# aws/karpenter-core

Measured on AMD Instinct MI355X. Metric: pod-placement decisions/sec (Solve()), higher is better.
Workload: dtype int64

## Files before the change

include/ksolve.h:

```cpp
#ifndef KSOLVE_H
#define KSOLVE_H
#include <stddef.h>
#include <stdint.h>

#ifdef __cplusplus
extern "C" {
#endif

#define KS_MAX_KEYS 32
#define KS_MAX_RES 16
#define KS_MAX_VALUES 64
#define KS_MAX_ITSTATES 65535
#define KS_NO_BOUND_GT INT32_MIN
#define KS_NO_BOUND_LT INT32_MAX
#define KS_KEY_HOSTNAME (-2)
#define KS_KEY_NONE (-1)

#define KS_OK 0
#define KS_ERR_INVALID (-1)
#define KS_ERR_UNSUPPORTED (-2)
#define KS_ERR_DEVICE (-3)
#define KS_ERR_CAPACITY (-4)
#define KS_ERR_INTERNAL (-5)

// ... 404 lines not shown
#define KS_CAND_WHY_DO_NOT_EVICT 12
#define KS_CAND_WHY_LEFT 13
typedef struct ks_candidates_inputs {
  uint32_t n_pods, n_nodes, n_pdbs, n_keys;
  const int32_t* pod_node;
  const uint32_t* pod_ns;
  const uint32_t* pod_flags;
  const double* pod_deletion_cost;
  const int32_t* pod_priority;
  const uint8_t* pod_val;
  const uint32_t* pdb_ns;
  const int32_t* pdb_allowed;
  const uint32_t* pdb_req_off;
  const uint32_t* pdb_req_key; const uint64_t* pdb_req_mask;
  const uint32_t* node_why;
  const double* node_age_seconds;
  const int64_t* node_ttl_seconds;
  const uint32_t* node_pods_off;
  const uint32_t* node_pods;
} ks_candidates_inputs;
typedef struct ks_candidates_outputs {
  uint32_t n_candidates, n_empty;
  uint32_t* order; uint32_t* empty; uint32_t* why; int32_t* detail; uint32_t* n_node_pods; double* cost;
} ks_candidates_outputs;
int ks_consolidation_candidates_host(const ks_candidates_inputs* in, ks_candidates_outputs* out, int device, double* ms );

#define KS_METHOD_EXPIRATION 1u
#define KS_METHOD_DRIFT 2u
#define KS_METHOD_EMPTINESS 3u
#define KS_DEPROV_WHY_NOT_EXPIRED 14
#define KS_DEPROV_WHY_NOT_DRIFTED 15
#define KS_DEPROV_WHY_NOT_EMPTY 16
#define KS_DEPROV_NODE_DELETION_TIMESTAMP 1u
#define KS_DEPROV_NODE_HAS_EMPTINESS 2u
#define KS_DEPROV_NODE_EMPTINESS_UNPARSABLE 4u
#define KS_DEPROV_NODE_DRIFTED 8u
#define KS_DEPROV_NODE_ALL 15u
#define KS_DEPROV_MAX_TTL_SECONDS 9223372036ll
typedef struct ks_deprov_inputs {
  ks_candidates_inputs c;
  uint32_t method, drift_enabled;
  int64_t now_unix_nanos;
  const uint32_t* node_dflags;
  const int64_t* node_creation_unix_nanos;
  const int64_t* node_emptiness_unix_nanos;
  const int64_t* node_ttl_seconds_after_empty;
} ks_deprov_inputs;
typedef struct ks_deprov_outputs { ks_candidates_outputs c; uint32_t n_in_result, pad; } ks_deprov_outputs;
int ks_deprovisioning_candidates_host(const ks_deprov_inputs* in, ks_deprov_outputs* out, int device, double* ms );

#define KS_CAND_VALUE_OTHER 0xFFFFFFFFu
#define KS_CAND_OP_IN 0u
#define KS_CAND_OP_NOT_IN 1u
#define KS_CAND_OP_EXISTS 2u
#define KS_CAND_OP_DOES_NOT_EXIST 3u
typedef struct ks_selector_lists {
  uint32_t n_keys, n_namespaces;
  const uint32_t* key_n_values;
  const uint32_t* pod_label_off;
  const uint32_t* pod_label_key;
  const uint32_t* pod_label_val;
  const uint32_t* req_key;
  const uint32_t* req_op;
  const uint32_t* req_val_off;
  const uint32_t* req_val;
} ks_selector_lists;
int ks_consolidation_candidates_lists_host(const ks_candidates_inputs* in, const ks_selector_lists* sel, ks_candidates_outputs* out, int device, double* ms );
int ks_deprovisioning_candidates_lists_host(const ks_deprov_inputs* in, const ks_selector_lists* sel, ks_deprov_outputs* out, int device, double* ms );

int ks_launch_pick_dev(ks_dev_problem* const* ds, uint32_t n, const uint32_t* node, int32_t* out_type, int32_t* out_pair, double* out_price);

int ks_types_subset_dev(ks_dev_problem* const* ds, uint32_t n, const uint32_t* node, const uint64_t* lhs, uint32_t stride_words, uint32_t* out);

typedef struct ks_req1 { uint64_t mask; int32_t gt, lt; uint8_t present, complement; } ks_req1;
int ks_probe_intersection(const ks_req1* a, const ks_req1* b, const int32_t* value_int, uint32_t nvalues, int on_device, ks_req1* out);
int ks_probe_compatible(const ks_req1* a, const ks_req1* b, int well_known, const int32_t* value_int, uint32_t nvalues, int on_device, int* ok);

typedef struct ks_req_facts { uint64_t has_mask; int64_t len; int32_t op; uint8_t nidne, len0; } ks_req_facts;
int ks_probe_has(const ks_req1* a, const int32_t* value_int, uint32_t nvalues, int on_device, ks_req_facts* out);

const char* ks_last_error(void);
const char* ks_version(void);
uint32_t ks_rr_run_max(void);

#ifdef __cplusplus
}
#endif
#endif
```

karpenter_core_amd/csrc/ks_pack_rr.inc:

```
#define KS_RR_DECLINED 0xDEC11EDull
#ifndef KS_SIM
#undef LSYNC
#define LSYNC() asm volatile("" ::: "memory")
#endif
#ifdef KS_PROBES
#define RRP(i) do { const u64 t_ = __builtin_readcyclecounter(); rrp[(i)] += t_ - rrp_t; rrp_t = t_; } while (0)
#else
#define RRP(i) do { } while (0)
#endif
#ifndef RR_NWK
#define RR_NWK 7
#endif
#define RR_NW (RR_NWK + 1)
#define RR_NPL 8
#define RR_NWN RR_NWK
#define RR_NODES (RR_NWN * 64 * RR_NPL)
#define RR_NODE_AT(slot, wk, ln) (((slot) * RR_NWN * 64u) + (u32)(ln) * RR_NWN + (wk))
#define RR_NODE_SLOT(n) ((n) / (64u * RR_NWN))
#define RR_NODE_WV(n) (((n) % (64u * RR_NWN)) % RR_NWN + 1u)
#define RR_NODE_LANE(n) (((n) % (64u * RR_NWN)) / RR_NWN)
#define RR_NRC 64
#define RR_GW 8
#define RR_KMAX 16
#define RR_HC_ZERO (RR_GW * 256u)
// ... 283 lines not shown
      for (u32 j = tl.topo_begin; j < tl.topo_end; ++j) {
        const PlanTopo& tg = c.topo[j]; const TopoDyn& d = sh.dyn[j]; u64 options = 0;
        if (d.reg == 0 && d.pos == ~0ull) continue;
        constrained = true;
        if (tg.type == 0) {
          i32 best = INT32_MAX; int bestv = -1;
          for (u64 bits = d.reg & ND; bits; bits &= bits - 1) {
            const int dd = __builtin_ctzll(bits);
            const i32 cnt = tb.gcnt[(size_t)tg.g * 64 + dd] + tg.self;
            if ((i64)cnt - (i64)d.minc <= (i64)tg.maxskew && cnt < best) { best = cnt; bestv = dd; }
          }
          if (bestv >= 0) options = 1ull << bestv;
        } else if (tg.type == 1) {
          options = d.reg & tg.PD & d.pos;
          if (!options && tg.self) {
            KReq pd = kreq_exists();
            if (tg.pod_has) { pd.present = true; pd.complement = tl.complement; pd.mask = tl.mask; pd.gt = KS_NOGT; pd.lt = KS_NOLT; }
            const u64 I = kreq_has_mask(kreq_intersect(pd, nd, vi, nv), vi, nv);
            const u64 x = d.reg & I, y = d.reg & tg.PD;
            if (x) options |= x & (~x + 1);
            if (y) options |= y & (~y + 1);
          }
        } else options = d.reg & tg.PD & ~d.pos;
        if (!options) return -KS_WHY_TOPOLOGY;
        dom &= options;
      }
      if (constrained) {
        const KReq in = kreq_in(dom);
        if (!before.present) { if (!((tb.wellknown >> k) & 1u)) return -KS_WHY_TOPOLOGY_REQS; a = in; }
        else { const KReq mg = kreq_intersect(in, before, vi, nv); if (kreq_len0(mg) && !kreq_nidne(before)) return -KS_WHY_TOPOLOGY_REQS; a = mg; }
      }
    }
    if (a.present) tpres |= 1u << i;
    if (a.complement) tcomp |= 1u << i;
    if (kreq_differs(a, orig)) tchg |= 1u << i;
    sh.la_mask[i][lane] = a.mask;
  }
  return 2;
}

#define RR_CTX \
  RRLds& L = g_rr_lds; \
  const DevProb& P = L.P; const DevState& S = L.S; WaveShared& sh = L.sh; RRNrc& nt = L.nt; LeaderShared& ls = L.ls; FastTabs& ft = L.ft; \
  Tabs tb; \
  tb.K = UF(P.K); tb.R = UF(P.R); tb.T = UF(P.T); tb.TW = UF(P.TW); tb.GH = UF(P.GH); tb.E = UF(P.E); tb.S = UF(P.S); tb.SC = UF(P.SC); tb.n_ct = UF(P.n_ct); tb.wellknown = UF(P.wellknown_mask); tb.key_zone = (i32)UF(P.key_zone); tb.key_ct = (i32)UF(P.key_ct); \
  tb.q = (GA u64*)UF64((u64)S.q); tb.pod_node = (GA i32*)UF64((u64)S.pod_node); tb.pod_seq = (GA i32*)UF64((u64)S.pod_seq); \
  tb.rec = (GA u8*)UF64((u64)S.rec); tb.rec_stride = UF(S.rec_stride); tb.hcnt = (GA i32*)UF64((u64)S.hcnt); tb.n_alive = (GA u64*)UF64((u64)S.n_alive); tb.ge_rows = (const GA u64*)UF64((u64)P.ge_rows); \
  const u32 nP = UF(P.P), nM = UF(P.M), nC = UF(P.C), nG = UF(P.G), nMAX = UF(P.NMAX), nE = tb.E, nK = tb.K, nR = tb.R, nTW = tb.TW; \
  i64* const ge = (i64*)ks_dyn_lds; const u32 gs = UF(P.ge_max); \
  tb.key_nvalues = ft.key_nvalues; tb.value_int = ft.value_int; tb.its_fail = ft.its_fail; tb.its_inter = ft.its_inter; \
  tb.gcnt = ft.gcnt; tb.g_reg = ft.g_reg; tb.g_pos = ft.g_pos; tb.g_active = ft.g_active; tb.g_hpos = ft.g_hpos; tb.g_hzero = ft.g_hzero; tb.ge_cnt = ft.ge_cnt; tb.ge_vals = ge; tb.ge_stride = gs; \
  const GA ClsPlan* const plans = (const GA ClsPlan*)UF64((u64)P.plans); \
  const GA u32* const rrb = (const GA u32*)UF64((u64)P.rr_briefs); \
  GA u32* const rrm = (GA u32*)UF64((u64)P.rr_memo); \
  GA u64* const rr_types = (GA u64*)UF64((u64)P.rr_types); \
  const GA u32* const rr_mi = (const GA u32*)UF64((u64)P.rr_mi); \
  (void)sh; (void)nt; (void)ls; (void)nP; (void)nM; (void)nC; (void)nG; (void)nMAX; (void)nK; (void)nR; (void)nTW; (void)plans; (void)rrb; (void)rrm; (void)rr_types; (void)rr_mi; (void)ge; (void)gs

__shared__ RRLds g_rr_lds;

__device__ __forceinline__ u32 rr_run_group(const u64* items, const int lane, const u32 done, const u32 rem, u32& item0, u32& item1) {
  const bool in = (u32)lane < rem;
  const u64 ab = in ? items[done + lane] : 0ull;
  const u32 a = (u32)ab, b = (u32)(ab >> 32);
  item0 = RL(a, 0); item1 = RL(b, 0);
  const u64 diff = ~ballot64(in && a == item0 && b == item1);
  return diff ? (u32)__builtin_ctzll(diff) : 64u;
}
#define RR_ITEM_LIM(p) ((i32)(((p) >> 16) & 0x1FFu) - (i32)((((p) >> 16) & 0x100u) << 1))

__device__ __forceinline__ u32 rr_step_merge(const u64 (*stepk)[8], u64* const scratch, const int lane, const u32 rem, const u32 nE, const u64 vfy, u32& o_key, u32& o_pay, u32& kind, u32& stop_node, u32& stop_nrc, u32& o_rank) {
  const u64 v = (u32)lane < RR_NWK * 8u ? stepk[lane >> 3][lane & 7] : ~0ull;
  const u32 key = (u32)(v >> 32);
  const bool valid = key != 0xFFFFFFFFu;
  o_key = 0xFFFFFFFFu; o_pay = 0; kind = 0; stop_node = 0xFFFFFFFFu; stop_nrc = 0;
  u32 rank = 0;
  { const u32* const kw = (const u32*)&stepk[0][0];
#pragma unroll 4
    for (u32 m = 0; m < RR_NWK * 8u; ++m) rank += kw[2u * m + 1u] < key ? 1u : 0u; }
  o_rank = valid ? rank : 64u;
  const u32 nvalid = (u32)__builtin_popcountll(ballot64(valid));
  if (rem == 0) return 0;
  if (nvalid == 0) { kind = 2; return 0; }
  if (valid) scratch[rank] = (v & ~(1ull << 31)) | (((u32)lane & 7u) == 7u ? (1ull << 31) : 0ull);
  LSYNC();
  const bool in = (u32)lane < nvalid;
  const u64 sv = in ? scratch[lane] : ~0ull;
  LSYNC();
  const u32 skey = (u32)(sv >> 32), spay = (u32)sv & 0x7FFFFFFFu, node = spay & 0xFFFFu, nrc = (spay >> 16) & 0xFFu;
  const u32 b0 = RL(skey, 0) >> 22;
  const bool h_b = (skey >> 22) != b0, h_c = node >= nE && (skey >> 22) >= RR_CNTMAX, h_v = ((vfy >> nrc) & 1ull) != 0;
  const u64 hb = ballot64(in && (h_b || h_c || h_v)), sb = ballot64(in && (node < nE || (((u32)sv >> 31) & 1u)));
  const u64 cb = ballot64(in && !h_b && h_c), vb = ballot64(in && !h_b && !h_c && h_v);
  const u32 cap = min(min((u32)RR_STEP, rem), nvalid);
  u32 n = cap;
  bool by_hard = false;
  if (hb) { const u32 t = (u32)__builtin_ctzll(hb); if (t < n) { n = t; by_hard = true; } }
  if (sb) { const u32 t = (u32)__builtin_ctzll(sb) + 1u; if (t <= n) { if (t < n || by_hard) by_hard = false; n = min(n, t); } }
  if (by_hard) { kind = ((cb >> n) & 1ull) ? 4u : (((vb >> n) & 1ull) ? 3u : 0u); if (kind) { stop_node = RL(node, (int)n); stop_nrc = RL(nrc, (int)n); } }
  if ((u32)lane < n) { o_key = skey; o_pay = spay; }
  return n;
}

__device__ __attribute__((noinline)) u32 rr_step_merge_leader(const u32 sp, const int lane, const u32 rem, const u32 nE, const u64 vfy) {
  RRLds& L = g_rr_lds;
  u32 wkey, wpay, kind, snode, snrc, mrank;
  const u32 n = rr_step_merge(L.stepk[sp], L.mrg[0], lane, rem, nE, vfy, wkey, wpay, kind, snode, snrc, mrank);
  L.mrg_out[lane] = wpay;
  if (lane == 0) { L.mrg_k[0] = kind; L.mrg_k[1] = snode; L.mrg_k[2] = snrc; }
  LSYNC();
  return n;
}

__device__ __forceinline__ u32 rr_pick_decide(const u32 nE, const u32 mw, const u64 w, u32& node, u32& nrc, u32& child, u32& key) {
  node = 0xFFFFFFFFu; nrc = 0; child = 0; key = 0;
  if (w == ~0ull) return 2u;
  node = (u32)w & 0xFFFFu; nrc = ((u32)w >> 16) & 0xFFu; key = (u32)(w >> 32);
  const u64 chg = (u64)RL(mw, 2) | ((u64)RL(mw, 3) << 32), vfy = (u64)RL(mw, 4) | ((u64)RL(mw, 5) << 32);
  child = ((chg >> nrc) & 1ull) ? ((RL(mw, 8 + (int)(nrc >> 2)) >> (8u * (nrc & 3u))) & 0xFFu) : nrc;
  if (node >= nE && (key >> 22) >= RR_CNTMAX) return 4u;
  if ((vfy >> nrc) & 1ull) return 3u;
  return 0u;
}

__device__ __forceinline__ void rr_px_static(const int lane, const u32 pos, const u32 nn, const u64 gam, const GA u32* const rrm) {
  RRLds& L = g_rr_lds; const RRNrc& nt = L.nt;
  RREntry& E = L.ring[pos & (RR_RING - 1u)]; RRPx& X = L.px[pos & (RR_PX - 1u)];
  if (lane == 0) RR_LDS_STORE(&X.u[0], 0xFFFFFFFFu);
  LSYNC();
  const u32x4 we = *(const u32x4*)&E.w[48];
  const u32x4 wq = *(const u32x4*)&E.w[52];
  const u32x4 wh = *(const u32x4*)&E.w[56];
  u32x4 m0 = *(const u32x4*)&E.t1[0], m1 = *(const u32x4*)&E.t1[4];
  const bool cover = we.x == pos && wq.x == 0 && (wq.z & 1u);
  if (UF((cover && m1.z < nn) ? 1u : 0u)) {
    const u32 mi = UF(wq.y); const u32 mw = (u32)lane < 24 ? rrm[(size_t)mi * 24 + lane] : 0u;
    LSYNC(); if ((u32)lane < 32) { E.m[lane] = mw; E.t1[lane] = mw; } LSYNC();
    m0 = *(const u32x4*)&E.t1[0]; m1 = *(const u32x4*)&E.t1[4];
  }
  const bool go = UF((cover && m1.z == nn) ? 1u : 0u) != 0;
  u32 flags = RR_PX_STOP7, dg = 0, ngrp = 0, ho = 0, plainb = 0xFFFFFFFFu, dself = 0, dskew = 0, dpd = 0;
  if (go) {
    const u32 it0 = wq.w, it1 = wh.x, hr0 = wh.y, hr1 = wh.z, nr0 = wh.w;
    const bool dyn = UF(wq.z & 2u) != 0;
    const bool cnt0 = ((hr0 >> 25) & 1u) && (((hr0 >> 24) & 1u) || ((gam >> ((hr0 >> 16) & 63u)) & 1ull)), cnt1 = ((hr1 >> 25) & 1u) && (((hr1 >> 24) & 1u) || ((gam >> ((hr1 >> 16) & 63u)) & 1ull));
    const u32 ho0 = cnt0 ? (hr0 & 0xFFFFu) : RR_HC_SINK, ho1 = cnt1 ? (hr1 & 0xFFFFu) : RR_HC_SINK;
    ho = ho0 | (ho1 << 16);
    plainb = (!dyn && (it0 & 0xFFFFu) == RR_HC_ZERO && (it1 & 0xFFFFu) == RR_HC_ZERO) ? E.w[27] : 0xFFFFFFFFu;
    flags = RR_PX_GO | (dyn ? RR_PX_DYN : 0u) | ((dyn || (m0.z | m0.w) != 0) ? RR_PX_CHG : 0u) | ((ho1 == ho0 && cnt0 && cnt1) ? RR_PX_TWICE : 0u) | ((cnt0 || cnt1) ? RR_PX_HREC : 0u);
    ngrp = nr0 & 63u;
    {
      const u32 n = (u32)lane;
      const u64 acc1 = (u64)m0.x | ((u64)m0.y << 32), chg1 = (u64)m0.z | ((u64)m0.w << 32), vfy1 = (u64)m1.x | ((u64)m1.y << 32);
      const u32 cbyte = ((const u8*)&E.t1[8])[n];
      const bool a_ok = n < nn && ((acc1 >> n) & 1ull), a_vfy = (vfy1 >> n) & 1ull; const u32 a_child = ((chg1 >> n) & 1ull) ? cbyte : n;
      const u32 nkey = (nr0 >> 8) & 0xFFu;
      auto rec_of = [&](const u32 ac) -> u32 {
        const u32 npres = nt.present[ac], ncomp = nt.complement[ac]; const u64 nqm = nt.mask[nkey & (RR_KMAX - 1u)][ac];
        const bool rec = ((nr0 >> 16) & 1u) && ((gam >> ngrp) & 1ull) && ((npres >> nkey) & 1u) && !((ncomp >> nkey) & 1u) && __builtin_popcountll(nqm) == 1;
        return rec ? (1u | ((u32)__builtin_ctzll(nqm | (1ull << 63)) << 1)) : 0u; };
      const u32 r0 = rec_of(a_child & 63u);
      u32 tw = (a_child & 0xFFu) | (a_ok ? 1u << 8 : 0u) | (a_vfy ? 1u << 9 : 0u) | ((r0 & 1u) << 11) | (((r0 >> 1) & 63u) << 12);
      if (dyn) {
        const u32 dw = E.w[11], dk = (dw >> 16) & 0xFFu, dk0 = UF(L.wx[8]), dk1 = UF(L.wx[9]);
        dg = (dw >> 8) & 63u; dself = dw >> 24; dskew = E.w[19]; dpd = E.w[26];
        const u32 dks = dk == dk0 ? 0u : 1u, n1 = a_child & 63u;
        const u64 nd = L.dy_nd[dks][n1], vp = L.vpair[n];
// ... 346 lines not shown
        const u32 kind = rr_pick_decide(nE, mw, w, node, nrc, nrc_new, key);
        if (kind != 0) { stop_kind = kind; stop_node = node; break; }
        pseq = seq0 + j; phm = UF(E.w[51]); pbp = E.w;
        RRP(13);
      }
      const u32 oslot = RR_NODE_SLOT(node), owv = RR_NODE_WV(node), olane = RR_NODE_LANE(node);
      if (owv == wv) {
        const bool mine = (u32)lane == olane;
        const u32 cbw = pbp[lane];
        if (it >= 0 && mine) { const u32 pd = pbp[50]; tb.pod_node[pd] = (i32)node; tb.pod_seq[pd] = (i32)pseq; G_pod_reason[pd] = 0;
        }
        const i64 cq0 = (i64)((u64)RL(cbw, 0) | ((u64)RL(cbw, 1) << 32)), cq1 = (i64)((u64)RL(cbw, 2) | ((u64)RL(cbw, 3) << 32)), cq2 = (i64)((u64)RL(cbw, 4) | ((u64)RL(cbw, 5) << 32)), cq3 = (i64)((u64)RL(cbw, 6) | ((u64)RL(cbw, 7) << 32));
        const u32 prm = RL(cbw, 8), nhrec = RL(cbw, 17);
        const u32* const crp = C.create;
        u32 rej = 0;
#define RR_HREC_WORD(i, w) case w: { const u32 c = (n_hc[i][w] >> sh8) & 0xFFu; const u32 c2 = c == 0xFFu ? 1u : (c >= 254u ? 254u : c + 1u); if (mine) { n_hc[i][w] = (n_hc[i][w] & ~(0xFFu << sh8)) | (c2 << sh8); if (c == 0u) hzm |= 1u << (hs & 31u); } } break;
#define RR_COMMIT_SLOT(i) if (oslot == (i)) { \
          if (create) { \
            if (mine) { n_key[i] = UF(crp[0]); n_meta[i] = nrc_new | (UF(crp[1]) << 8); \
              n_room[i][0] = (i64)((u64)UF(crp[2]) | ((u64)UF(crp[3]) << 32)); n_room[i][1] = (i64)((u64)UF(crp[4]) | ((u64)UF(crp[5]) << 32)); \
              n_room[i][2] = (i64)((u64)UF(crp[6]) | ((u64)UF(crp[7]) << 32)); n_room[i][3] = (i64)((u64)UF(crp[8]) | ((u64)UF(crp[9]) << 32)); \
              n_hc[i][0] = UF(crp[10]); n_hc[i][1] = UF(crp[11]); n_hc[i][2] = UF(crp[12]); n_hc[i][3] = UF(crp[13]); n_hc[i][4] = UF(crp[14]); n_hc[i][5] = UF(crp[15]); n_hc[i][6] = UF(crp[16]); n_hc[i][7] = UF(crp[17]); } \
          } else { \
            const u32 nrc_old = RL(n_meta[i], (int)olane) & 0xFFu; \
            i64 d0 = cq0, d1 = cq1, d2 = cq2, d3 = cq3; \
            if (node >= nE && nrc_new != nrc_old) { d0 -= nt.cap[0][nrc_new] - nt.cap[0][nrc_old]; d1 -= nt.cap[1][nrc_new] - nt.cap[1][nrc_old]; d2 -= nt.cap[2][nrc_new] - nt.cap[2][nrc_old]; d3 -= nt.cap[3][nrc_new] - nt.cap[3][nrc_old]; } \
            if (mine) { \
              n_room[i][0] -= d0; n_room[i][1] -= d1; n_room[i][2] -= d2; n_room[i][3] -= d3; \
              if (node >= nE) n_key[i] = (((n_key[i] >> 22) + 1u) << 22) | ((RR_SEQMAX - pseq) << 3) | (n_key[i] & 7u); \
              n_meta[i] = nrc_new | ((((n_meta[i] >> 8) | prm) & 0xFFu) << 8); } \
          } \
          for (u32 t = 0; t < nhrec; ++t) if ((phm >> t) & 1u) {        \
            const u32 hs = RL(cbw, 28 + (int)t) & 0xFFu, sh8 = 8u * (hs & 3u); \
            switch (hs >> 2) { RR_HREC_WORD(i, 0) RR_HREC_WORD(i, 1) RR_HREC_WORD(i, 2) RR_HREC_WORD(i, 3) RR_HREC_WORD(i, 4) RR_HREC_WORD(i, 5) RR_HREC_WORD(i, 6) RR_HREC_WORD(i, 7) default: break; } \
          } \
          if (it >= 0) { RR_EVAL_SLOT(i) \
            if (nhost > 0) RR_HOST_ITEM(RR_HOST_AT_##i, hit0, hlim0) if (nhost > 1) RR_HOST_ITEM(RR_HOST_AT_##i, hit1, hlim1) if (nhost > 2) RR_HOST_ITEM(RR_HOST_AT_##i, hit2, hlim2) \
            okm = (okm & ~(1u << (i))) | (~rej & (1u << (i))); fresh = true; } }
#define RR_HOST_AT_0(w, sh, lim) RR_HOST_SLOT(0, w, sh, lim)
#define RR_HOST_AT_1(w, sh, lim) RR_HOST_SLOT(1, w, sh, lim)
#define RR_HOST_AT_2(w, sh, lim) RR_HOST_SLOT(2, w, sh, lim)
#define RR_HOST_AT_3(w, sh, lim) RR_HOST_SLOT(3, w, sh, lim)
#define RR_HOST_AT_4(w, sh, lim) RR_HOST_SLOT(4, w, sh, lim)
#define RR_HOST_AT_5(w, sh, lim) RR_HOST_SLOT(5, w, sh, lim)
#define RR_HOST_AT_6(w, sh, lim) RR_HOST_SLOT(6, w, sh, lim)
#define RR_HOST_AT_7(w, sh, lim) RR_HOST_SLOT(7, w, sh, lim)
        RR_COMMIT_SLOT(0) RR_COMMIT_SLOT(1) RR_COMMIT_SLOT(2) RR_COMMIT_SLOT(3) RR_COMMIT_SLOT(4) RR_COMMIT_SLOT(5) RR_COMMIT_SLOT(6) RR_COMMIT_SLOT(7)
        RR_HZ_FLUSH()
      }
    }
    if (run) {
      const RREntry& E = L.ring[pos0 & (RR_RING - 1u)];
      const u32 mw = E.m[lane & 31];
      do_eval(E, mw, 0u, true);
      u32 okb = okm, cur_item = 0, cur_item1 = 0;
      const u32 rbw = E.w[lane];
      const u32 rprm = RL(rbw, 8);
      const u64 rchg = (u64)RL(mw, 2) | ((u64)RL(mw, 3) << 32), rvfy = (u64)RL(mw, 4) | ((u64)RL(mw, 5) << 32);
      u32 done = 0, stepno = 0;
#ifdef KS_PROBES
      const u64 trun0 = __builtin_readcyclecounter(); u64 tx = trun0;
#define RRT(i) do { const u64 t_ = __builtin_readcyclecounter(); rrp[(i)] += t_ - tx; tx = t_; } while (0)
#else
#define RRT(i) do { } while (0)
#endif
      RRT(0);
      while (done < run) {
        u32 g_i0, g_i1;
        const u32 glen = rr_run_group(L.runitem[par], lane, done, run - done, g_i0, g_i1);
        RRT(5);
        if (g_i0 != cur_item || g_i1 != cur_item1) {
          cur_item = g_i0; cur_item1 = g_i1; nhost = (g_i0 >> 31) + (g_i1 >> 31);
          hit0 = g_i0 & 0xFFFFu; hlim0 = RR_ITEM_LIM(g_i0); hit1 = g_i1 & 0xFFFFu; hlim1 = RR_ITEM_LIM(g_i1);
          u32 rej = 0;
          if (nhost > 0) RR_HOST_ITEM(RR_HOST_ALL, hit0, hlim0)
          if (nhost > 1) RR_HOST_ITEM(RR_HOST_ALL, hit1, hlim1)
          okm = okb & ~rej;
        }
        RRT(6);
        const u32 rem = min(run - done, glen), sp = stepno & 1u;
        u32 kk[RR_NPL];
#pragma unroll
        for (int i = 0; i < RR_NPL; ++i) kk[i] = n_key[i] | (u32)(((i32)((okm >> i) & 1u)) - 1);
        u32 myk = 0xFFFFFFFFu, mypay = 0, b0 = 0;
        RRT(7);
        for (u32 r = 0; r < 8u && r < rem; ++r) {
          u32 lb = kk[0];
#pragma unroll
          for (int i = 1; i < RR_NPL; ++i) lb = min(lb, kk[i]);
          const u32 km = wave_min_u32(lb);
          if (km == 0xFFFFFFFFu) break;
          if (r == 0) b0 = km >> 22; else if ((km >> 22) != b0) break;
          const int wl = __builtin_ctzll(ballot64(lb == km));
          const u32 ws = km & 7u;
          u32 bm = 0;
#pragma unroll
          for (int i = 0; i < RR_NPL; ++i) if ((u32)i == ws) bm = n_meta[i];
          const u32 nd = RR_NODE_AT(ws, wk_i, wl);
          const u32 bmu = RL(bm, wl);
          if ((u32)lane == r) { myk = km; mypay = ((bmu & 0xFFu) << 16) | nd; }
#pragma unroll
          for (int i = 0; i < RR_NPL; ++i) if ((u32)i == ws) kk[i] = lane == wl ? 0xFFFFFFFFu : kk[i];
          if (nd < nE) break;
        }
        if (lane < 8) L.stepk[sp][wk_i][lane] = ((u64)myk << 32) | mypay;
        RRT(1);
        __syncthreads();
        RRT(2);
        u32 wkey, wpay, kind, snode, snrc;
        u32 mrank;
        const u32 n_step = rr_step_merge(L.stepk[sp], L.mrg[wv], lane, rem, nE, rvfy, wkey, wpay, kind, snode, snrc, mrank);
        RRT(3);
        u32 ts = 0;
        for (u32 r = 0; r < 8u; ++r) {
          const u32 j = RL(mrank, (int)(wk_i * 8u + r));
          if (j >= n_step) break;
          const u32 pay = UF((u32)L.stepk[sp][wk_i][r]), node = pay & 0xFFFFu, nrc = (pay >> 16) & 0xFFu;
          const u32 oslot = RR_NODE_SLOT(node), olane = RR_NODE_LANE(node);
          const u32 nrc_new = ((rchg >> nrc) & 1ull) ? ((RL(mw, 8 + (int)(nrc >> 2)) >> (8u * (nrc & 3u))) & 0xFFu) : nrc;
          const bool mine = (u32)lane == olane;
          const u32 rpw = lane < 6 ? ((const u32*)&L.runtab[par][done + j])[lane] : 0u;
          const u32 pseq = seq0 + done + j, nh = RL(rpw, 2), pd = RL(rpw, 0);
          if (mine) { tb.pod_node[pd] = (i32)node; tb.pod_seq[pd] = (i32)pseq; G_pod_reason[pd] = 0;
          }
          ts |= 1u << oslot;
#define RR_RCOMMIT_SLOT(i) if (oslot == (i)) { \
            i64 d0 = rq0, d1 = rq1, d2 = rq2, d3 = rq3; \
            if (node >= nE && nrc_new != nrc) { d0 -= nt.cap[0][nrc_new] - nt.cap[0][nrc]; d1 -= nt.cap[1][nrc_new] - nt.cap[1][nrc]; d2 -= nt.cap[2][nrc_new] - nt.cap[2][nrc]; d3 -= nt.cap[3][nrc_new] - nt.cap[3][nrc]; } \
            if (mine) { \
              n_room[i][0] -= d0; n_room[i][1] -= d1; n_room[i][2] -= d2; n_room[i][3] -= d3; \
              if (node >= nE) n_key[i] = (((n_key[i] >> 22) + 1u) << 22) | ((RR_SEQMAX - pseq) << 3) | (n_key[i] & 7u); \
              n_meta[i] = nrc_new | ((((n_meta[i] >> 8) | rprm) & 0xFFu) << 8); } \
            for (u32 t = 0; t < nh; ++t) {        \
              const u32 hs = (RL(rpw, 3 + (int)(t >> 2)) >> (8u * (t & 3u))) & 0xFFu, sh8 = 8u * (hs & 3u); \
              switch (hs >> 2) { RR_HREC_WORD(i, 0) RR_HREC_WORD(i, 1) RR_HREC_WORD(i, 2) RR_HREC_WORD(i, 3) RR_HREC_WORD(i, 4) RR_HREC_WORD(i, 5) RR_HREC_WORD(i, 6) RR_HREC_WORD(i, 7) default: break; } \
            } }
          RR_RCOMMIT_SLOT(0) RR_RCOMMIT_SLOT(1) RR_RCOMMIT_SLOT(2) RR_RCOMMIT_SLOT(3) RR_RCOMMIT_SLOT(4) RR_RCOMMIT_SLOT(5) RR_RCOMMIT_SLOT(6) RR_RCOMMIT_SLOT(7)
        }
        RR_HZ_FLUSH()
        if (ts) {
          u32 rej = 0, rejh = 0;
#define RR_RETRY_SLOT(i) if ((ts >> (i)) & 1u) { RR_EVAL_SLOT(i) }
          RR_RETRY_SLOT(0) RR_RETRY_SLOT(1) RR_RETRY_SLOT(2) RR_RETRY_SLOT(3) RR_RETRY_SLOT(4) RR_RETRY_SLOT(5) RR_RETRY_SLOT(6) RR_RETRY_SLOT(7)
          okb = (okb & ~ts) | (~rej & ts);
          if (nhost) { rej = 0;
#define RR_RETRYH_SLOT(i) if ((ts >> (i)) & 1u) { RR_HOST_ITEM(RR_HOST_AT_##i, hit0, hlim0) if (nhost > 1) RR_HOST_ITEM(RR_HOST_AT_##i, hit1, hlim1) }
            RR_RETRYH_SLOT(0) RR_RETRYH_SLOT(1) RR_RETRYH_SLOT(2) RR_RETRYH_SLOT(3) RR_RETRYH_SLOT(4) RR_RETRYH_SLOT(5) RR_RETRYH_SLOT(6) RR_RETRYH_SLOT(7)
            rejh = rej; }
          okm = (okm & ~ts) | (okb & ~rejh & ts);
        }
        RRT(4);
        done += n_step; ++stepno;
        if (kind != 0) { stop_kind = kind; stop_node = snode; break; }
      }
    }
    if (stop_kind == 3) {
      const u32 oslot = RR_NODE_SLOT(stop_node), owv = RR_NODE_WV(stop_node), olane = RR_NODE_LANE(stop_node);
      if (owv == wv) {
        u32 bmeta = 0; i64 broom[4] = {0, 0, 0, 0};
#pragma unroll
        for (int i = 0; i < RR_NPL; ++i) if ((u32)i == oslot) { bmeta = n_meta[i]; broom[0] = n_room[i][0]; broom[1] = n_room[i][1]; broom[2] = n_room[i][2]; broom[3] = n_room[i][3]; }
        if ((u32)lane == olane) { L.ask.meta = bmeta; L.ask.room[0] = broom[0]; L.ask.room[1] = broom[1]; L.ask.room[2] = broom[2]; L.ask.room[3] = broom[3]; }
      }
      __syncthreads();
    }
    if (RL(hdw, RRH_HINT)) { const u32 ql = RL(hdw, RRH_QL); pf_n = ql > nb ? min(ql - nb, RR_RING - 2u) : 0u; pf_pos = pos0 + nb; pf_qi = RL(hdw, RRH_QH) + nb; pf_gam = (u64)RL(hdw, RRH_GAM) | ((u64)RL(hdw, RRH_GAM + 1) << 32); }
    RRP(14);
    ++round;
  }
  {
    GA u64* const dump = (GA u64*)P.rr_nodes;
#pragma unroll
    for (int i = 0; i < RR_NPL; ++i) {
      const u32 n = RR_NODE_AT((u32)i, wk_i, lane);
      if (n_key[i] != 0xFFFFFFFFu && n >= nE) { dump[(size_t)n * 5] = n_meta[i]; for (int r = 0; r < 4; ++r) dump[(size_t)n * 5 + 1 + r] = (u64)n_room[i][r]; }
    }
    __threadfence_block(); GSYNC();
  }
#if defined(KS_SIM) || defined(KS_CHECK)
#pragma unroll
  for (int i = 0; i < RR_NPL; ++i) if (n_key[i] != 0xFFFFFFFFu) for (u32 h = 0; h < tb.GH; ++h) {
    u32 b = 1;
#pragma unroll
    for (int w = 0; w < RR_GW; ++w) if ((h >> 2) == (u32)w) b = (n_hc[i][w] >> (8 * (h & 3u))) & 0xFFu;
    if (b == 0u) atomicAdd(&L.hz[h & 31u], -1);
  }
#endif
#ifdef KS_PROBES
  if (wv == 1 && lane == 0) for (int i = 0; i < 16; ++i) L.wst[i] = rrp[i];
#endif
}

__device__ __attribute__((noinline)) void rr_build_types(const int lane, const u32 id) {
  RR_CTX;
    const i32 m = (i32)UF((u32)nt.tmpl[id]); const u32 pres = UF(nt.present[id]), comp = UF(nt.complement[id]); const i32 its = (i32)UF((u32)nt.it[id]);
    u64 allowZ = ~0ull, allowC = ~0ull;
    if (tb.key_zone >= 0 && ((pres >> tb.key_zone) & 1u)) { KReq z; z.present = true; z.complement = (comp >> tb.key_zone) & 1u; z.mask = nt.mask[tb.key_zone][id]; z.gt = KS_NOGT; z.lt = KS_NOLT; allowZ = kreq_has_mask(z, tb.value_int + tb.key_zone * 64, tb.key_nvalues[tb.key_zone]); }
    if (tb.key_ct >= 0 && ((pres >> tb.key_ct) & 1u)) { KReq z; z.present = true; z.complement = (comp >> tb.key_ct) & 1u; z.mask = nt.mask[tb.key_ct][id]; z.gt = KS_NOGT; z.lt = KS_NOLT; allowC = kreq_has_mask(z, tb.value_int + tb.key_ct * 64, tb.key_nvalues[tb.key_ct]); }
    for (u32 wbase = 0; wbase < nTW; wbase += 64) {
      const u32 w = wbase + lane;
      if (w < nTW) {
        u64 a = GC(u64, P.tmpl_types)[(size_t)m * nTW + w] & G_its_types[(size_t)its * nTW + w];
        for (u32 bits = pres; bits; bits &= bits - 1) {
          const int k = __builtin_ctz(bits);
          KReq B; B.present = true; B.complement = (comp >> k) & 1u; B.mask = nt.mask[k][id]; B.gt = KS_NOGT; B.lt = KS_NOLT;
          a &= pass_types_word(P, tb, k, B, w);
        }
        if (tb.n_ct != 0) {
          u64 acc = 0; const u64 cm = allowC & ((1ull << tb.n_ct) - 1);
          for (u64 zz = allowZ; zz; zz &= zz - 1) { const int z = __builtin_ctzll(zz); if ((u32)z * tb.n_ct >= 64) break; for (u64 cb = cm; cb; cb &= cb - 1) acc |= G_pair_types[((size_t)z * tb.n_ct + __builtin_ctzll(cb)) * nTW + w]; }
          a &= acc;
        }
        rr_types[(size_t)id * nTW + w] = a;
      }
    }
    GSYNC();
    i64 mx[4];
#pragma unroll
    for (int r = 0; r < 4; ++r) mx[r] = INT64_MIN;
// ... 1305 lines not shown
```

karpenter_core_amd/csrc/ksolve.hip:

```cpp
#include <hip/hip_runtime.h>

#include <cmath>
#include <cstdio>
#include <cstdlib>
#include <algorithm>
#include <cstring>
#include <string>
#include <vector>
#include <type_traits>
#include <system_error>

#include "../../include/ksolve.h"
#include "ks_algebra.h"

#define KS_FLAG_NOFOLD 0x10000u
#define KS_MAX_TOPO 24
#define KS_MAX_TOUCH 12
#define KS_RES_NARROW 8
#define KS_LEAN8_NW 4

#ifdef KS_SIM
struct u32x4 { unsigned int x, y, z, w; };
#else
typedef unsigned int u32x4 __attribute__((ext_vector_type(4)));
// ... 4061 lines not shown
  const size_t o_lhs = st.add<u64>((size_t)n * stride_words), o_node = st.add<u32>(n), o_out = st.add<u32>(n);
  TRY(st.place());
  memcpy(st.h<u64>(o_lhs), lhs, (size_t)n * stride_words * sizeof(u64)); memcpy(st.h<u32>(o_node), node, n * sizeof(u32));
  TRY(st.upload(o_out));
  hipLaunchKernelGGL(ks_types_subset, dim3(n), dim3(64), 0, st.stream(), st.probs(), st.states(), st.d<const u32>(o_node), st.d<const u64>(o_lhs), stride_words, st.d<u32>(o_out));
  TRY(st.fetch(o_out));
  memcpy(out, st.h<u32>(o_out), n * sizeof(u32));
  return KS_OK;
}

extern "C" int ks_solve_dev(ks_dev_problem* d, ks_result* out, float* kernel_ms) {
  if (!d || !out) return fail(KS_ERR_INVALID, "null argument");
  ks_dev_problem* arr[1] = {d}; ks_result* outs[1] = {out};
  return ks_solve_batch_dev(arr, 1, outs, kernel_ms);
}

extern "C" int ks_solve(const ks_problem* p, ks_result* out) {
  ks_dev_problem* d = nullptr;
  TRY(ks_problem_upload(p, 0, &d));
  int rc = ks_solve_dev(d, out, nullptr);
  ks_problem_free(d); return rc;
}

extern "C" int ks_solve_batch(const ks_problem* const* ps, uint32_t n, ks_result* const* outs) {
  std::vector<ks_dev_problem*> ds(n, nullptr); int rc = KS_OK;
  for (u32 i = 0; i < n && rc == KS_OK; ++i) rc = ks_problem_upload(ps[i], 0, &ds[i]);
  if (rc == KS_OK) rc = ks_solve_batch_dev(ds.data(), n, outs, nullptr);
  for (auto* d : ds) ks_problem_free(d);
  return rc;
}

static KReq to_k(const ks_req1* a) { KReq r; r.mask = a->mask; r.gt = a->gt; r.lt = a->lt; r.present = a->present; r.complement = a->complement; return r; }
static void from_k(const KReq& r, ks_req1* o) { o->mask = r.mask; o->gt = r.gt; o->lt = r.lt; o->present = r.present; o->complement = r.complement; }

static int probe_device(const ks_req1* a, const ks_req1* b, int wk, const int32_t* vint, uint32_t nv, ks_req1* out, int* ok) {
  if (ks_device_count() <= 0) return fail(KS_ERR_DEVICE, "no gfx950 device");
  i32* dv; ks_req1* dout; int* dok;
  HIPCHK(hipMalloc((void**)&dv, 64 * sizeof(i32))); HIPCHK(hipMalloc((void**)&dout, sizeof(ks_req1))); HIPCHK(hipMalloc((void**)&dok, sizeof(int)));
  i32 tmp[64]; for (int i = 0; i < 64; ++i) tmp[i] = (u32)i < nv ? vint[i] : INT32_MIN;
  HIPCHK(hipMemcpy(dv, tmp, sizeof tmp, hipMemcpyHostToDevice));
  hipLaunchKernelGGL(ks_probe_kernel, dim3(1), dim3(1), 0, 0, *a, *b, dv, nv, wk, dout, dok);
  HIPCHK(hipDeviceSynchronize());
  if (out) HIPCHK(hipMemcpy(out, dout, sizeof(ks_req1), hipMemcpyDeviceToHost));
  if (ok) HIPCHK(hipMemcpy(ok, dok, sizeof(int), hipMemcpyDeviceToHost));
  hipFree(dv); hipFree(dout); hipFree(dok); return KS_OK;
}

extern "C" int ks_probe_intersection(const ks_req1* a, const ks_req1* b, const int32_t* value_int, uint32_t nvalues, int on_device, ks_req1* out) {
  if (on_device) return probe_device(a, b, 1, value_int, nvalues, out, nullptr);
  from_k(kreq_intersect(to_k(a), to_k(b), value_int, nvalues), out); return KS_OK;
}
extern "C" int ks_probe_compatible(const ks_req1* a, const ks_req1* b, int well_known, const int32_t* value_int, uint32_t nvalues, int on_device, int* ok) {
  if (on_device) return probe_device(a, b, well_known, value_int, nvalues, nullptr, ok);
  *ok = !kreq_compatible_fail(to_k(a), to_k(b), well_known != 0, value_int, nvalues); return KS_OK;
}

extern "C" int ks_probe_has(const ks_req1* a, const int32_t* value_int, uint32_t nvalues, int on_device, ks_req_facts* out) {
  if (!a || !out || !value_int) return fail(KS_ERR_INVALID, "null argument");
  if (!on_device) { ks_req_facts_of(to_k(a), value_int, nvalues, out); return KS_OK; }
  if (ks_device_count() <= 0) return fail(KS_ERR_DEVICE, "no gfx950 device");
  int device = ks_current_device(); TmpDev tv(device), to(device);
  TRY(tv.alloc(64 * sizeof(i32))); TRY(to.alloc(sizeof(ks_req_facts)));
  i32 tmp[64]; for (int i = 0; i < 64; ++i) tmp[i] = (u32)i < nvalues ? value_int[i] : INT32_MIN;
  HIPCHK(hipMemcpy(tv.p, tmp, sizeof tmp, hipMemcpyHostToDevice));
  const i32* dv = tv.as<i32>(); ks_req_facts* dout = to.as<ks_req_facts>();
  hipLaunchKernelGGL(ks_probe_has_kernel, dim3(1), dim3(1), 0, 0, *a, dv, nvalues, dout);
  HIPCHK(hipDeviceSynchronize());
  HIPCHK(hipMemcpy(out, to.p, sizeof(ks_req_facts), hipMemcpyDeviceToHost));
  return KS_OK;
}

extern "C" int ks_debug_classes(ks_dev_problem* d, void* briefs_out, void* plans_out) {
  if (!d) return fail(KS_ERR_INVALID, "null device problem");
  if (!d->tables_built) TRY(build_static(d, nullptr));
  HIPCHK(hipSetDevice(d->device));
  if (briefs_out) HIPCHK(hipMemcpy(briefs_out, d->h.briefs, (size_t)d->h.C * sizeof(ClsBrief), hipMemcpyDeviceToHost));
  if (plans_out) HIPCHK(hipMemcpy(plans_out, d->h.plans, (size_t)d->h.C * sizeof(ClsPlan), hipMemcpyDeviceToHost));
  return (int)sizeof(ClsPlan);
}

extern "C" const char* ks_last_error(void) { return g_err.c_str(); }
extern "C" const char* ks_version(void) { return "ksolve 0.1.0 (gfx950)"; }
extern "C" uint32_t ks_rr_run_max(void) { return RR_RUN_MAX; }
```

Measured before the change: 964,500.

## Publish same-bucket step candidates in one ballot pass and slot-indexed commit

The per-wave candidate selection for each packing step used to extract up to eight minimum keys one at a time, each with a wave-wide min reduction. It now publishes every candidate in the leading count bucket at once, using ballots and prefix popcounts, whenever that bucket holds eight or fewer entries. Otherwise it falls back to the serial loop. The commit loop now iterates only over the slots that were published, using a recorded slot-to-rank map instead of re-reading payloads from shared memory, and it reads hostname records with byte loads. It also adds a small build-flag query function for probe builds. The reworked bit encoding and key-update conditions (b0 != 0 in place of node >= nE) carry a risk of subtle correctness changes.

```diff
diff --git a/include/ksolve.h b/include/ksolve.h
--- a/include/ksolve.h
+++ b/include/ksolve.h
@@ -510,6 +510,10 @@
 const char* ks_last_error(void);
 const char* ks_version(void);
 uint32_t ks_rr_run_max(void);
+#define KS_PROBE_BUILD_PROBES 1u
+#define KS_PROBE_BUILD_WIN 2u
+#define KS_PROBE_BUILD_RUN 4u
+uint32_t ks_probe_build(void);
 
 #ifdef __cplusplus
 }
diff --git a/karpenter_core_amd/csrc/ks_pack_rr.inc b/karpenter_core_amd/csrc/ks_pack_rr.inc
--- a/karpenter_core_amd/csrc/ks_pack_rr.inc
+++ b/karpenter_core_amd/csrc/ks_pack_rr.inc
@@ -389,7 +389,7 @@
   const u32 nvalid = (u32)__builtin_popcountll(ballot64(valid));
   if (rem == 0) return 0;
   if (nvalid == 0) { kind = 2; return 0; }
-  if (valid) scratch[rank] = (v & ~(1ull << 31)) | (((u32)lane & 7u) == 7u ? (1ull << 31) : 0ull);
+  if (valid) scratch[rank] = v;
   LSYNC();
   const bool in = (u32)lane < nvalid;
   const u64 sv = in ? scratch[lane] : ~0ull;
@@ -902,28 +902,58 @@
         u32 kk[RR_NPL];
 #pragma unroll
         for (int i = 0; i < RR_NPL; ++i) kk[i] = n_key[i] | (u32)(((i32)((okm >> i) & 1u)) - 1);
-        u32 myk = 0xFFFFFFFFu, mypay = 0, b0 = 0;
         RRT(7);
-        for (u32 r = 0; r < 8u && r < rem; ++r) {
-          u32 lb = kk[0];
-#pragma unroll
-          for (int i = 1; i < RR_NPL; ++i) lb = min(lb, kk[i]);
-          const u32 km = wave_min_u32(lb);
-          if (km == 0xFFFFFFFFu) break;
-          if (r == 0) b0 = km >> 22; else if ((km >> 22) != b0) break;
-          const int wl = __builtin_ctzll(ballot64(lb == km));
-          const u32 ws = km & 7u;
-          u32 bm = 0;
-#pragma unroll
-          for (int i = 0; i < RR_NPL; ++i) if ((u32)i == ws) bm = n_meta[i];
-          const u32 nd = RR_NODE_AT(ws, wk_i, wl);
-          const u32 bmu = RL(bm, wl);
-          if ((u32)lane == r) { myk = km; mypay = ((bmu & 0xFFu) << 16) | nd; }
-#pragma unroll
-          for (int i = 0; i < RR_NPL; ++i) if ((u32)i == ws) kk[i] = lane == wl ? 0xFFFFFFFFu : kk[i];
-          if (nd < nE) break;
-        }
-        if (lane < 8) L.stepk[sp][wk_i][lane] = ((u64)myk << 32) | mypay;
+        u32 lb = kk[0];
+#pragma unroll
+        for (int i = 1; i < RR_NPL; ++i) lb = min(lb, kk[i]);
+        u32 km = wave_min_u32(lb);
+        const u32 b0 = km >> 22;
+        u32 pubw = 0, pubm = 0;
+        bool one_by_one = true;
+        if (km != 0xFFFFFFFFu && b0 != 0u) {
+          u64 mb[RR_NPL]; u32 total = 0;
+#pragma unroll
+          for (int i = 0; i < RR_NPL; ++i) { mb[i] = ballot64(kk[i] != 0xFFFFFFFFu && (kk[i] >> 22) == b0); total += (u32)__builtin_popcountll(mb[i]); }
+          if (total <= 8u) {
+            one_by_one = false;
+            const u64 below = (1ull << lane) - 1ull;
+            u32 base = 0;
+#pragma unroll
+            for (int i = 0; i < RR_NPL; ++i) {
+              if ((mb[i] >> lane) & 1ull) {
+                const u32 pl = base + (u32)__builtin_popcountll(mb[i] & below);
+                L.stepk[sp][wk_i][pl] = ((u64)kk[i] << 32) | (u64)(((n_meta[i] & 0xFFu) << 16) | RR_NODE_AT((u32)i, wk_i, lane));
+                pubw |= (1u << i) | (pl << (8 + 3 * i));
+              }
+              base += (u32)__builtin_popcountll(mb[i]); pubm |= mb[i] ? 1u << i : 0u;
+            }
+            if (lane < 8 && (u32)lane >= total) L.stepk[sp][wk_i][lane] = ~0ull;
+          }
+        }
+        if (one_by_one) {
+          u32 myk = 0xFFFFFFFFu, mypay = 0;
+          if (km != 0xFFFFFFFFu) for (u32 r = 0;;) {
+            const int wl = __builtin_ctzll(ballot64(lb == km));
+            const u32 ws = km & 7u;
+            u32 bm = 0;
+#pragma unroll
+            for (int i = 0; i < RR_NPL; ++i) if ((u32)i == ws) bm = n_meta[i];
+            const u32 nd = RR_NODE_AT(ws, wk_i, wl);
+            const u32 bmu = RL(bm, wl);
+            if ((u32)lane == r) { myk = km; mypay = ((bmu & 0xFFu) << 16) | nd | (r == 7u ? 1u << 31 : 0u); }
+            if (lane == wl) pubw |= (1u << ws) | (r << (8u + 3u * ws));
+            pubm |= 1u << ws;
+            if (b0 == 0u || ++r >= 8u || r >= rem) break;
+#pragma unroll
+            for (int i = 0; i < RR_NPL; ++i) if ((u32)i == ws) kk[i] = lane == wl ? 0xFFFFFFFFu : kk[i];
+            lb = kk[0];
+#pragma unroll
+            for (int i = 1; i < RR_NPL; ++i) lb = min(lb, kk[i]);
+            km = wave_min_u32(lb);
+            if (km == 0xFFFFFFFFu || (km >> 22) != b0) break;
+          }
+          if (lane < 8) L.stepk[sp][wk_i][lane] = ((u64)myk << 32) | mypay;
+        }
         RRT(1);
         __syncthreads();
         RRT(2);
@@ -932,29 +962,28 @@
         const u32 n_step = rr_step_merge(L.stepk[sp], L.mrg[wv], lane, rem, nE, rvfy, wkey, wpay, kind, snode, snrc, mrank);
         RRT(3);
         u32 ts = 0;
-        for (u32 r = 0; r < 8u; ++r) {
-          const u32 j = RL(mrank, (int)(wk_i * 8u + r));
-          if (j >= n_step) break;
-          const u32 pay = UF((u32)L.stepk[sp][wk_i][r]), node = pay & 0xFFFFu, nrc = (pay >> 16) & 0xFFu;
-          const u32 oslot = RR_NODE_SLOT(node), olane = RR_NODE_LANE(node);
-          const u32 nrc_new = ((rchg >> nrc) & 1ull) ? ((RL(mw, 8 + (int)(nrc >> 2)) >> (8u * (nrc & 3u))) & 0xFFu) : nrc;
-          const bool mine = (u32)lane == olane;
-          const u32 rpw = lane < 6 ? ((const u32*)&L.runtab[par][done + j])[lane] : 0u;
-          const u32 pseq = seq0 + done + j, nh = RL(rpw, 2), pd = RL(rpw, 0);
-          if (mine) { tb.pod_node[pd] = (i32)node; tb.pod_seq[pd] = (i32)pseq; G_pod_reason[pd] = 0;
-          }
+        for (u32 sb = pubm; sb; sb &= sb - 1u) {
+          const u32 oslot = (u32)__builtin_ctz(sb);
+          const u32 j = __shfl(mrank, (int)(wk_i * 8u + ((pubw >> (8u + 3u * oslot)) & 7u)));
+          const bool mine = ((pubw >> oslot) & 1u) != 0u && j < n_step;
+          if (!ballot64(mine)) continue;
           ts |= 1u << oslot;
+          const u32* const rpw = (const u32*)&L.runtab[par][done + (mine ? j : 0u)];
+          const u32 pseq = seq0 + done + j, nh = mine ? rpw[2] : 0u;
+          if (mine) { const u32 pd = rpw[0]; tb.pod_node[pd] = (i32)RR_NODE_AT(oslot, wk_i, (u32)lane); tb.pod_seq[pd] = (i32)pseq; G_pod_reason[pd] = 0; }
 #define RR_RCOMMIT_SLOT(i) if (oslot == (i)) { \
-            i64 d0 = rq0, d1 = rq1, d2 = rq2, d3 = rq3; \
-            if (node >= nE && nrc_new != nrc) { d0 -= nt.cap[0][nrc_new] - nt.cap[0][nrc]; d1 -= nt.cap[1][nrc_new] - nt.cap[1][nrc]; d2 -= nt.cap[2][nrc_new] - nt.cap[2][nrc]; d3 -= nt.cap[3][nrc_new] - nt.cap[3][nrc]; } \
+            const u32 nrc = n_meta[i] & 0xFFu, chw = rchg ? __shfl(mw, (int)(8u + ((nrc >> 2) & 15u))) : 0u;       \
             if (mine) { \
-              n_room[i][0] -= d0; n_room[i][1] -= d1; n_room[i][2] -= d2; n_room[i][3] -= d3; \
-              if (node >= nE) n_key[i] = (((n_key[i] >> 22) + 1u) << 22) | ((RR_SEQMAX - pseq) << 3) | (n_key[i] & 7u); \
-              n_meta[i] = nrc_new | ((((n_meta[i] >> 8) | rprm) & 0xFFu) << 8); } \
-            for (u32 t = 0; t < nh; ++t) {        \
-              const u32 hs = (RL(rpw, 3 + (int)(t >> 2)) >> (8u * (t & 3u))) & 0xFFu, sh8 = 8u * (hs & 3u); \
-              switch (hs >> 2) { RR_HREC_WORD(i, 0) RR_HREC_WORD(i, 1) RR_HREC_WORD(i, 2) RR_HREC_WORD(i, 3) RR_HREC_WORD(i, 4) RR_HREC_WORD(i, 5) RR_HREC_WORD(i, 6) RR_HREC_WORD(i, 7) default: break; } \
-            } }
+              const u32 nrc_new = ((rchg >> nrc) & 1ull) ? ((chw >> (8u * (nrc & 3u))) & 0xFFu) : nrc; \
+              n_room[i][0] -= rq0; n_room[i][1] -= rq1; n_room[i][2] -= rq2; n_room[i][3] -= rq3; \
+              if (b0 != 0u) { \
+                n_key[i] = (((n_key[i] >> 22) + 1u) << 22) | ((RR_SEQMAX - pseq) << 3) | (n_key[i] & 7u); \
+                if (nrc_new != nrc) { n_room[i][0] += nt.cap[0][nrc_new] - nt.cap[0][nrc]; n_room[i][1] += nt.cap[1][nrc_new] - nt.cap[1][nrc]; n_room[i][2] += nt.cap[2][nrc_new] - nt.cap[2][nrc]; n_room[i][3] += nt.cap[3][nrc_new] - nt.cap[3][nrc]; } } \
+              n_meta[i] = nrc_new | ((((n_meta[i] >> 8) | rprm) & 0xFFu) << 8); \
+              for (u32 t = 0; t < nh; ++t) {        \
+                const u32 hs = ((const u8*)rpw)[12u + t], sh8 = 8u * (hs & 3u); \
+                switch (hs >> 2) { RR_HREC_WORD(i, 0) RR_HREC_WORD(i, 1) RR_HREC_WORD(i, 2) RR_HREC_WORD(i, 3) RR_HREC_WORD(i, 4) RR_HREC_WORD(i, 5) RR_HREC_WORD(i, 6) RR_HREC_WORD(i, 7) default: break; } \
+              } } }
           RR_RCOMMIT_SLOT(0) RR_RCOMMIT_SLOT(1) RR_RCOMMIT_SLOT(2) RR_RCOMMIT_SLOT(3) RR_RCOMMIT_SLOT(4) RR_RCOMMIT_SLOT(5) RR_RCOMMIT_SLOT(6) RR_RCOMMIT_SLOT(7)
         }
         RR_HZ_FLUSH()
diff --git a/karpenter_core_amd/csrc/ksolve.hip b/karpenter_core_amd/csrc/ksolve.hip
--- a/karpenter_core_amd/csrc/ksolve.hip
+++ b/karpenter_core_amd/csrc/ksolve.hip
@@ -4167,3 +4167,16 @@
 extern "C" const char* ks_last_error(void) { return g_err.c_str(); }
 extern "C" const char* ks_version(void) { return "ksolve 0.1.0 (gfx950)"; }
 extern "C" uint32_t ks_rr_run_max(void) { return RR_RUN_MAX; }
+extern "C" uint32_t ks_probe_build(void) {
+  uint32_t f = 0;
+#ifdef KS_PROBES
+  f |= KS_PROBE_BUILD_PROBES;
+#endif
+#ifdef KS_PROBES_WIN
+  f |= KS_PROBE_BUILD_WIN;
+#endif
+#ifdef KS_PROBES_RUN
+  f |= KS_PROBE_BUILD_RUN;
+#endif
+  return f;
+}
```

After: 1.016 million (median of 6 runs). +5.3%, better.
